# VKCOM/YouTokenToMe

Hardware: NVIDIA B200
Metric: encode throughput, 1M x 128 B synthetic sentences, vocab 32k (higher is better)
Workload: dtype u8/u32

## Files before the change

youtokentome_b200/csrc/encode.cu:

```cuda
#include <algorithm>
#include <cstdlib>
#include <cstring>

#include "common.cuh"

using namespace yt;

namespace {

constexpr int32_t EMPTY_SLOT = -1;
constexpr uint32_t NO_RANK = 0xffffffffu;

struct RuleTab {
  const uint4 *slots;
  uint32_t mask;
};

__device__ __forceinline__ uint32_t rule_rank(const RuleTab &rt, uint32_t a, uint32_t b, uint32_t *z) {
  if ((a | b) & UNK_FLAG) return NO_RANK;
  uint32_t h = rule_hash(a, b) & rt.mask;
  while (true) {
    uint4 s = __ldg(rt.slots + h);
    if (s.x == a && s.y == b) { *z = s.w; return s.z; }
    if (s.x == 0xffffffffu) return NO_RANK;
    h = (h + 1) & rt.mask;
  }
}

struct EncArgs {
  const uint8_t *bytes;
  const uint64_t *offs;
  uint64_t n_sent;
  int32_t *slots;
  uint32_t *ranks;
  uint32_t *aux;
  uint32_t *word_pos;
  uint32_t *word_sent;
// ... 134 lines not shown
  }
}

constexpr int FIND_VEC_CACHE = 8;
__device__ __forceinline__ uint32_t find_vec_word(const uint8_t *s, int64_t p, int64_t lo, int64_t hi, int64_t n_total) {
  if (p + 4 <= lo) return 0x20202020u;
  if (p >= hi) return 0u;
  uint32_t w = 0;
  if (p >= 0 && p + 4 <= n_total) w = *reinterpret_cast<const uint32_t *>(s + p);
  else
    for (int k = 0; k < 4; k++)
      if (p + k >= 0 && p + k < n_total) w |= (uint32_t)s[p + k] << (8 * k);
  if (p < lo || p + 4 > hi)
    for (int k = 0; k < 4; k++) {
      if (p + k < lo) w = (w & ~(0xffu << (8 * k))) | (0x20u << (8 * k));
      else if (p + k >= hi) w &= ~(0xffu << (8 * k));
    }
  return w;
}
__device__ __forceinline__ uint32_t swar_eq(uint32_t w, uint32_t v4) {
  const uint32_t t = w ^ v4;
  return ~(((t & 0x7f7f7f7fu) + 0x7f7f7f7fu) | t | 0x7f7f7f7fu);
}
__device__ __forceinline__ uint32_t swar_space(uint32_t w) {
  const uint32_t b7 = w & 0x7f7f7f7fu;
  const uint32_t ge9 = b7 + 0x77777777u, ge14 = b7 + 0x72727272u;
  return (swar_eq(w, 0x20202020u) | (ge9 & ~ge14 & ~w)) & 0x80808080u;
}
__device__ __forceinline__ uint32_t swar_mask4(uint32_t hi) {
  const uint32_t m = hi >> 7;
  return (m | (m >> 7) | (m >> 14) | (m >> 21)) & 15u;
}
__device__ __forceinline__ uint32_t find_vec_flags(const uint8_t *s, int64_t p, int64_t lo, int64_t hi, int64_t n_total,
                                                   unsigned lane) {
  const uint32_t c = find_vec_word(s, p, lo, hi, n_total);
  uint32_t pv = __shfl_up_sync(0xffffffffu, c, 1), nx = __shfl_down_sync(0xffffffffu, c, 1);
  if (lane == 0) pv = find_vec_word(s, p - 4, lo, hi, n_total);
  if (lane == 31) nx = find_vec_word(s, p + 4, lo, hi, n_total);
  uint32_t inside = 15u;
  if (p < lo) inside &= lo - p >= 4 ? 0u : 15u << (uint32_t)(lo - p);
  if (p + 4 > hi) inside &= hi <= p ? 0u : 15u >> (uint32_t)(p + 4 - hi);
  if (!((swar_eq(pv, 0xe2e2e2e2u) | swar_eq(c, 0xe2e2e2e2u) | swar_eq(nx, 0xe2e2e2e2u)) & 0x80808080u)) {
    const uint32_t sp = swar_mask4(swar_space(c)), sp_prev = swar_mask4(swar_space(pv)) >> 3;
    return ((sp << 1) | sp_prev) & ~sp & inside & 15u;
  }
  const uint64_t X = (uint64_t)pv | ((uint64_t)c << 32), Y = (uint64_t)c | ((uint64_t)nx << 32);
  uint32_t f = 0;
#pragma unroll
  for (int k = 0; k < 4; k++) {
    const uint32_t t = (uint32_t)(X >> (8 * (1 + k))), u = (uint32_t)(Y >> (8 * k));
    const bool before = is_space_byte((uint8_t)(t >> 16)) || (t & 0xffffffu) == 0x8196e2u;
    const bool at = is_space_byte((uint8_t)u) || (u & 0xffffffu) == 0x8196e2u;
    if (before && !at) f |= 1u << k;
  }
  return f & inside;
}
constexpr int FIND_SPW = 4;
__global__ void __launch_bounds__(256) find_words_vec_kernel(EncArgs a) {
  __shared__ unsigned long long s_cnt[8 * FIND_SPW], s_base;
  const unsigned lane = threadIdx.x & 31, wid = threadIdx.x >> 5;
  const uint64_t o0 = a.offs[0];
  const int64_t n_total = (int64_t)(a.offs[a.n_sent] - o0);
  const int64_t mis = (int64_t)(reinterpret_cast<uintptr_t>(a.bytes) & 3u);
  constexpr uint64_t PER_ROUND = 8 * FIND_SPW;
  for (uint64_t g = (uint64_t)blockIdx.x * PER_ROUND; g < a.n_sent; g += (uint64_t)gridDim.x * PER_ROUND) {
    int64_t lo[FIND_SPW], hi[FIND_SPW], start[FIND_SPW];
    uint32_t cnt[FIND_SPW];
    uint32_t cache = 0;
    constexpr int CPS = FIND_VEC_CACHE / FIND_SPW;
#pragma unroll
    for (int q = 0; q < FIND_SPW; q++) {
      const uint64_t s = g + (uint64_t)wid * FIND_SPW + q;
      lo[q] = hi[q] = start[q] = 0;
      cnt[q] = 0;
      if (s < a.n_sent) {
        lo[q] = (int64_t)(a.offs[s] - o0);
        hi[q] = (int64_t)(a.offs[s + 1] - o0);
        start[q] = lo[q] - ((lo[q] + mis) & 3);
        uint32_t mine = 0;
        int j = 0;
        for (int64_t pw = start[q]; pw < hi[q]; pw += 128, j++) {
          const uint32_t f = find_vec_flags(a.bytes, pw + 4 * lane, lo[q], hi[q], n_total, lane);
          if (j < CPS) cache |= f << (4 * (q * CPS + j));
          mine += __popc(f);
        }
        for (int o = 16; o > 0; o >>= 1) mine += __shfl_xor_sync(0xffffffffu, mine, o);
        cnt[q] = mine;
        if (lane == 0 && !a.direct) {
          const uint64_t base = sent_base((uint64_t)lo[q], s), len = (uint64_t)(hi[q] - lo[q]);
          a.n_ids[s] = (a.bos ? 1 : 0) + (a.eos ? 1 : 0);
          if (a.bos) a.slots[base] = a.bos_id;
          if (a.eos) a.slots[base + len + 2] = a.eos_id;
        }
      }
      if (lane == 0) s_cnt[wid * FIND_SPW + q] = cnt[q];
    }
    __syncthreads();
    if (wid == 0) {
      const unsigned long long c = s_cnt[lane];
      unsigned long long x = c;
      for (int o = 1; o < 32; o <<= 1) {
        const unsigned long long y = __shfl_up_sync(0xffffffffu, x, o);
        if ((int)lane >= o) x += y;
      }
      s_cnt[lane] = x - c;
      if (lane == 31) s_base = x ? atomicAdd(a.n_words, x) : 0ull;
    }
    __syncthreads();
#pragma unroll
    for (int q = 0; q < FIND_SPW; q++) {
      const uint64_t s = g + (uint64_t)wid * FIND_SPW + q;
      if (s >= a.n_sent) continue;
      unsigned long long idx = s_base + s_cnt[wid * FIND_SPW + q];
      if (lane == 0 && a.direct) { a.sent_wbase[s] = (uint32_t)idx; a.sent_wcnt[s] = cnt[q]; }
      if (!cnt[q]) continue;
      const unsigned below = (1u << lane) - 1u;
      int j = 0;
      for (int64_t pw = start[q]; pw < hi[q]; pw += 128, j++) {
        const int64_t p = pw + 4 * lane;
        const uint32_t f = j < CPS ? (cache >> (4 * (q * CPS + j))) & 15u : find_vec_flags(a.bytes, p, lo[q], hi[q], n_total, lane);
        const unsigned b0 = __ballot_sync(0xffffffffu, f & 1u), b1 = __ballot_sync(0xffffffffu, f & 2u),
                       b2 = __ballot_sync(0xffffffffu, f & 4u), b3 = __ballot_sync(0xffffffffu, f & 8u);
        const unsigned all_below = __popc(b0 & below) + __popc(b1 & below) + __popc(b2 & below) + __popc(b3 & below);
        unsigned long long i = idx + all_below;
#pragma unroll
        for (int k = 0; k < 4; k++)
          if ((f >> k) & 1u) {
            a.word_pos[i] = (uint32_t)(p + k);
            a.word_sent[i] = (uint32_t)s;
            i++;
          }
        idx += __popc(b0) + __popc(b1) + __popc(b2) + __popc(b3);
      }
    }
    __syncthreads();
  }
}

template <bool DROPOUT>
__global__ void __launch_bounds__(128) encode_words_kernel(EncArgs a, uint64_t n_words) {
  constexpr uint32_t LOCAL_W = 40;
  const uint64_t stride = (uint64_t)gridDim.x * blockDim.x;
  const uint64_t o0 = a.offs[0];
  const RuleTab rt = a.rt;
  auto rank = [&](uint32_t x, uint32_t y, uint32_t *z) { return rule_rank(rt, x, y, z); };
  for (uint64_t w = (uint64_t)blockIdx.x * blockDim.x + threadIdx.x; w < n_words; w += stride) {
    const uint64_t p0 = a.word_pos[w], s = a.word_sent[w];
    const uint64_t lo = a.offs[s] - o0, hi = a.offs[s + 1] - o0;
    const uint64_t slot0 = sent_base(lo, s) + 1 + (p0 - lo);
    int32_t *t = a.slots + slot0;
    uint64_t q = p0;
    uint32_t l;
    while (q < hi && !space_at(a.bytes, q, hi, &l)) q++;
// ... 249 lines not shown
      }
    }
    if (!no_unit && a.space_id == 0) {
      const bool drop = t[0] == 0;
      __syncthreads();
      if (drop) {
        for (uint32_t b0 = 0; b0 + 1 < n; b0 += LONG_T) {
          const uint32_t i = b0 + threadIdx.x;
          const uint32_t v = i + 1 < n ? t[i + 1] : 0u;
          __syncthreads();
          if (i + 1 < n) t[i] = v;
          __syncthreads();
        }
        n -= 1;
      }
    }
    const uint32_t n_out = no_unit ? 0 : n;
    for (uint32_t i = threadIdx.x; i < (a.direct ? n_out : owned); i += LONG_T) {
      const uint32_t v = t[i];
      t[i] = i < n_out ? ((v & UNK_FLAG) ? (uint32_t)a.unk_id : v) : (uint32_t)EMPTY_SLOT;
    }
    if (threadIdx.x == 0) {
      if (n_out && !a.direct) atomicAdd(a.n_ids + s, (unsigned long long)n_out);
      if (ll.n_tok) ll.n_tok[ll.item[w]] = n_out;
    }
    __syncthreads();
  }
}

constexpr unsigned long long DEDUP_EMPTY = ~0ull;
constexpr uint32_t DEDUP_PROBES = 8;
struct DedupArgs {
  unsigned long long *tab;
  uint32_t mask;
  uint32_t *rep;
  uint32_t *n_tok;
  uint32_t *list;
  unsigned long long *n_list;
  uint32_t weak_tag;
};

__global__ void __launch_bounds__(128) dedup_words_kernel(EncArgs a, uint64_t n_words, DedupArgs d) {
  const unsigned lane = threadIdx.x & 31;
  const uint64_t stride = (uint64_t)gridDim.x * blockDim.x;
  const uint64_t o0 = a.offs[0];
  for (uint64_t w0 = (uint64_t)blockIdx.x * blockDim.x + (threadIdx.x & ~31u); w0 < n_words; w0 += stride) {
    const uint64_t w = w0 + lane;
    bool is_rep = false;
    if (w < n_words) {
      const uint64_t p0 = a.word_pos[w], hi = a.offs[(uint64_t)a.word_sent[w] + 1] - o0;
      uint64_t q = p0, h = 0xcbf29ce484222325ull;
      uint32_t l;
      while (q < hi && !space_at(a.bytes, q, hi, &l)) { h = (h ^ a.bytes[q]) * 0x100000001b3ull; q++; }
      const uint64_t len = q - p0;
      h = mix64(h);
      const uint32_t tag = d.weak_tag ? 7u : (uint32_t)(h >> 32);
      const unsigned long long mine = ((unsigned long long)tag << 32) | (uint32_t)w;
      uint32_t idx = (uint32_t)h & d.mask, r = (uint32_t)w;
      is_rep = true;
      for (uint32_t k = 0; k < DEDUP_PROBES; k++, idx = (idx + 1) & d.mask) {
        unsigned long long cur = *(volatile unsigned long long *)(d.tab + idx);
        if (cur == DEDUP_EMPTY) {
          cur = atomicCAS(d.tab + idx, DEDUP_EMPTY, mine);
          if (cur == DEDUP_EMPTY) break;
        }
        if ((uint32_t)(cur >> 32) != tag) continue;
        const uint32_t w2 = (uint32_t)cur;
        const uint64_t p2 = a.word_pos[w2], hi2 = a.offs[(uint64_t)a.word_sent[w2] + 1] - o0;
        bool same = true;
        for (uint64_t i = 0; i < len; i++)
          if (p2 + i >= hi2 || a.bytes[p2 + i] != a.bytes[p0 + i]) { same = false; break; }
        if (same && p2 + len < hi2 && !space_at(a.bytes, p2 + len, hi2, &l)) same = false;
        if (same) { r = w2; is_rep = false; break; }
      }
      d.rep[w] = r;
    }
    const unsigned m = __ballot_sync(0xffffffffu, is_rep);
    if (m) {
      unsigned long long base = 0;
      if (lane == 0) base = atomicAdd(d.n_list, (unsigned long long)__popc(m));
      base = __shfl_sync(0xffffffffu, base, 0);
      if (is_rep) d.list[base + __popc(m & ((1u << lane) - 1))] = (uint32_t)w;
    }
  }
}

__global__ void __launch_bounds__(128) encode_rep_words_kernel(EncArgs a, DedupArgs d, LongList ll) {
  constexpr uint32_t LOCAL_W = 40;
  const uint64_t stride = (uint64_t)gridDim.x * blockDim.x;
  const uint64_t o0 = a.offs[0];
  const RuleTab rt = a.rt;
  auto rank = [&](uint32_t x, uint32_t y, uint32_t *z) { return rule_rank(rt, x, y, z); };
  const unsigned long long n_list = *d.n_list;
  for (uint64_t i = (uint64_t)blockIdx.x * blockDim.x + threadIdx.x; i < n_list; i += stride) {
    const uint32_t w = d.list[i];
    const uint64_t p0 = a.word_pos[w], s = a.word_sent[w];
    const uint64_t lo = a.offs[s] - o0, hi = a.offs[s + 1] - o0;
    const uint64_t slot0 = p0 + 3 * s + 1;
    int32_t *t = a.slots + slot0;
    uint64_t q = p0;
    uint32_t l;
    while (q < hi && !space_at(a.bytes, q, hi, &l)) q++;
    uint32_t owned = (uint32_t)(q - p0) + 1, n;
    if (ll.cap && owned > LONG_W) {
      const unsigned long long k = atomicAdd(ll.n, 1ull);
      if (k < ll.cap) { ll.pos[k] = (uint32_t)p0; ll.sent[k] = (uint32_t)s; ll.end[k] = (uint32_t)q; ll.item[k] = w; continue; }
    }
    if (owned <= LOCAL_W) {
      int32_t lt[LOCAL_W];
      uint32_t lr[LOCAL_W];
      n = encode_word(a.bytes, p0, lo, hi, a.cp2id, a.space_id, rank, nullptr, 0, a.seed, a.first_sentence + s, lt, lr,
                      nullptr, &owned);
      for (uint32_t k = 0; k < n; k++) t[k] = ((uint32_t)lt[k] & UNK_FLAG) ? a.unk_id : lt[k];
    } else {
      n = encode_word(a.bytes, p0, lo, hi, a.cp2id, a.space_id, rank, nullptr, 0, a.seed, a.first_sentence + s, t,
                      a.ranks + slot0, nullptr, &owned);
      for (uint32_t k = 0; k < n; k++)
        if ((uint32_t)t[k] & UNK_FLAG) t[k] = a.unk_id;
      if (!a.direct)
        for (uint32_t k = n; k < owned; k++) t[k] = EMPTY_SLOT;
    }
    d.n_tok[w] = n;
    if (n && !a.direct) atomicAdd(a.n_ids + s, (unsigned long long)n);
  }
}

__global__ void __launch_bounds__(256) copy_word_ids_kernel(EncArgs a, uint64_t n_words, DedupArgs d) {
  const uint64_t stride = (uint64_t)gridDim.x * blockDim.x;
  for (uint64_t w = (uint64_t)blockIdx.x * blockDim.x + threadIdx.x; w < n_words; w += stride) {
    const uint32_t r = d.rep[w];
    if (r == (uint32_t)w) continue;
    const uint32_t n = d.n_tok[r];
    if (!n) continue;
    const uint64_t s = a.word_sent[w];
    const int32_t *src = a.slots + ((uint64_t)a.word_pos[r] + 3ull * a.word_sent[r] + 1);
    int32_t *dst = a.slots + ((uint64_t)a.word_pos[w] + 3ull * s + 1);
    for (uint32_t k = 0; k < n; k++) dst[k] = src[k];
    atomicAdd(a.n_ids + s, (unsigned long long)n);
  }
}

__global__ void __launch_bounds__(256) sentence_ids_kernel(EncArgs a, const uint32_t *__restrict__ rep) {
  const unsigned lane = threadIdx.x & 31;
  const uint64_t warp = ((uint64_t)blockIdx.x * blockDim.x + threadIdx.x) >> 5;
  const uint64_t nwarps = ((uint64_t)gridDim.x * blockDim.x) >> 5;
  for (uint64_t s = warp; s < a.n_sent; s += nwarps) {
    const uint32_t w0 = a.sent_wbase[s], nw = a.sent_wcnt[s];
    uint32_t sum = 0;
    for (uint32_t i = lane; i < nw; i += 32) {
      const uint32_t w = w0 + i;
      sum += a.n_tok[rep ? rep[w] : w];
    }
    for (int o = 16; o > 0; o >>= 1) sum += __shfl_xor_sync(0xffffffffu, sum, o);
    if (lane == 0) a.n_ids[s] = (unsigned long long)sum + (a.bos ? 1 : 0) + (a.eos ? 1 : 0);
  }
}

__global__ void __launch_bounds__(256) emit_ids_kernel(EncArgs a, const uint32_t *__restrict__ rep,
                                                       const unsigned long long *__restrict__ out_off, int32_t *__restrict__ out) {
  const unsigned lane = threadIdx.x & 31;
  const uint64_t warp = ((uint64_t)blockIdx.x * blockDim.x + threadIdx.x) >> 5;
  const uint64_t nwarps = ((uint64_t)gridDim.x * blockDim.x) >> 5;
  for (uint64_t s = warp; s < a.n_sent; s += nwarps) {
    const uint32_t w0 = a.sent_wbase[s], nw = a.sent_wcnt[s];
    const unsigned long long ob = out_off[s], total = a.n_ids[s];
    auto at = [&](unsigned long long j) { return ob + (a.reverse ? total - 1 - j : j); };
    if (lane == 0) {
      if (a.bos) out[at(0)] = a.bos_id;
      if (a.eos) out[at(total - 1)] = a.eos_id;
    }
    unsigned long long pos = a.bos ? 1 : 0;
    for (uint32_t i0 = 0; i0 < nw; i0 += 32) {
      const uint32_t i = i0 + lane;
      uint32_t r = 0, n = 0;
      if (i < nw) {
        r = rep ? rep[w0 + i] : w0 + i;
        n = a.n_tok[r];
      }
      uint32_t x = n;
      for (int o = 1; o < 32; o <<= 1) {
        const uint32_t y = __shfl_up_sync(0xffffffffu, x, o);
        if ((int)lane >= o) x += y;
      }
      const uint32_t all = __shfl_sync(0xffffffffu, x, 31);
      if (n) {
        const int32_t *src = a.slots + ((uint64_t)a.word_pos[r] + 3ull * a.word_sent[r] + 1);
        const unsigned long long first = pos + (x - n);
        for (uint32_t k = 0; k < n; k++) out[at(first + k)] = src[k];
      }
      pos += all;
    }
  }
}

__global__ void __launch_bounds__(256) gather_ids_kernel(EncArgs a, const unsigned long long *__restrict__ out_off,
                                                         int32_t *__restrict__ out) {
  const unsigned lane = threadIdx.x & 31;
  const uint64_t warp = ((uint64_t)blockIdx.x * blockDim.x + threadIdx.x) >> 5;
  const uint64_t nwarps = ((uint64_t)gridDim.x * blockDim.x) >> 5;
  const uint64_t o0 = a.offs[0];
  for (uint64_t s = warp; s < a.n_sent; s += nwarps) {
    const uint64_t lo = a.offs[s] - o0, len = a.offs[s + 1] - o0 - lo;
    const uint64_t base = sent_base(lo, s);
    const unsigned long long ob = out_off[s], cnt = a.n_ids[s];
    unsigned long long done = 0;
    for (uint64_t i0 = 0; i0 < len + 3; i0 += 32) {
      uint64_t i = i0 + lane;
      int32_t v = i < len + 3 ? a.slots[base + i] : EMPTY_SLOT;
      unsigned m = __ballot_sync(0xffffffffu, v != EMPTY_SLOT);
      if (v != EMPTY_SLOT) {
        unsigned long long k = done + __popc(m & ((1u << lane) - 1));
        out[ob + (a.reverse ? cnt - 1 - k : k)] = v;
      }
      done += __popc(m);
    }
  }
}

__global__ void __launch_bounds__(256) add_base_kernel(unsigned long long *__restrict__ off, uint64_t n, unsigned long long base) {
// ... 39 lines not shown
  const uint64_t max_words = n_bytes / 2 + n_sent + 8;
  YT_CUDA(c, e->wpos.reserve(max_words * 4));
  YT_CUDA(c, e->wsent.reserve(max_words * 4));
  YT_CUDA(c, e->nids.reserve((n_sent + 1) * 8));
  YT_CUDA(c, e->out_off.reserve((n_sent + 2) * 8));
  YT_CUDA(c, e->counter.reserve(64));
  YT_CUDA(c, cudaMemsetAsync(e->counter.p, 0, 64, c->stream));
  EncArgs a;
  a.bytes = d_bytes; a.offs = d_offs; a.n_sent = n_sent;
  a.slots = e->slots.as<int32_t>(); a.ranks = e->ranks.as<uint32_t>();
  a.aux = dropout > 0 ? e->aux.as<uint32_t>() : nullptr;
  a.word_pos = e->wpos.as<uint32_t>(); a.word_sent = e->wsent.as<uint32_t>();
  a.n_words = e->counter.as<unsigned long long>();
  a.n_ids = e->nids.as<unsigned long long>();
  a.cp2id = enc->cp2id.as<uint32_t>();
  a.rt.slots = enc->rules.as<uint4>(); a.rt.mask = enc->rule_mask;
  a.space_id = enc->space_id;
  a.unk_id = enc->unk; a.bos_id = enc->bos; a.eos_id = enc->eos;
  a.bos = bos; a.eos = eos; a.reverse = reverse;
  a.drop_thresh = dropout <= 0 ? 0 : (uint64_t)(dropout * 4294967296.0);
  a.seed = seed; a.first_sentence = first_sentence;
  *out_n = 0;
  auto *d_total = e->counter.as<unsigned long long>() + 1;
  if (n_sent == 0) return 0;
  ytc::timer_begin(c, "encode");
  const bool plain = std::getenv("YTTM_ENC_PLAIN") != nullptr;
  const bool zlin = enc->zlin_ok && std::getenv("YTTM_ENC_ZLIN") != nullptr;
  const bool want_bucketed = std::getenv("YTTM_ENC_BUCKETED") != nullptr;
  const bool dedup = a.drop_thresh == 0 && (std::getenv("YTTM_ENC_DEDUP") != nullptr || (!plain && !zlin && !want_bucketed));
  const bool longw = a.drop_thresh == 0 && (std::getenv("YTTM_ENC_LONG") != nullptr || !plain);
  const bool bucketed = !dedup && (zlin || want_bucketed || (longw && std::getenv("YTTM_ENC_LONG") != nullptr));
  const bool find_vec = std::getenv("YTTM_ENC_FIND_VEC") || !(plain || std::getenv("YTTM_ENC_FIND_CACHED"));
  const bool direct = find_vec && !plain && !bucketed && !std::getenv("YTTM_ENC_SLOTS") && !std::getenv("YTTM_ENC_FIND_CACHED");
  a.direct = direct ? 1 : 0;
  a.sent_wbase = a.sent_wcnt = a.n_tok = nullptr;
  if (direct) {
    YT_CUDA(c, e->swb.reserve((n_sent + 1) * 4));
    YT_CUDA(c, e->swc.reserve((n_sent + 1) * 4));
    a.sent_wbase = e->swb.as<uint32_t>();
    a.sent_wcnt = e->swc.as<uint32_t>();
  }
  {
    ytc::timer_begin(c, "enc_find");
    if (!direct) YT_CUDA(c, cudaMemsetAsync(a.slots, 0xff, n_slots * 4, c->stream));
    if (find_vec) {
      const uint64_t blocks = std::min<uint64_t>((n_sent + 8 * FIND_SPW - 1) / (8 * FIND_SPW), (uint64_t)c->n_sm * 8);
      find_words_vec_kernel<<<(unsigned)std::max<uint64_t>(blocks, 1), 256, 0, c->stream>>>(a);
    } else {
      const uint64_t blocks = std::min<uint64_t>((n_sent + 7) / 8, (uint64_t)c->n_sm * 8);
      if (std::getenv("YTTM_ENC_FIND_CACHED")) find_words_cached_kernel<<<(unsigned)std::max<uint64_t>(blocks, 1), 256, 0, c->stream>>>(a);
      else find_words_kernel<<<(unsigned)std::max<uint64_t>(blocks, 1), 256, 0, c->stream>>>(a);
    }
    ytc::timer_end(c, "enc_find");
    c->launches++;
  }
  unsigned long long n_words = 0;
  YT_CUDA(c, cudaMemcpyAsync(&n_words, a.n_words, 8, cudaMemcpyDeviceToHost, c->stream));
  YT_CUDA(c, cudaStreamSynchronize(c->stream));
  const uint32_t *d_rep = nullptr;
  if (n_words) {
    uint64_t blocks = std::min<uint64_t>((n_words + 127) / 128, (uint64_t)c->n_sm * 16);
    ytc::timer_begin(c, "enc_words");
    LongList ll{nullptr, nullptr, nullptr, nullptr, nullptr, nullptr, 0};
    if (longw && (dedup || bucketed)) {
      const uint32_t cap = (uint32_t)(n_bytes / LONG_W + 16);
      YT_CUDA(c, e->longw.reserve((size_t)cap * 16 + 16));
      ll.n = e->longw.as<unsigned long long>();
      ll.pos = reinterpret_cast<uint32_t *>(ll.n + 2);
      ll.sent = ll.pos + cap;
      ll.end = ll.sent + cap;
      ll.item = ll.end + cap;
      ll.cap = cap;
      YT_CUDA(c, cudaMemsetAsync(ll.n, 0, 8, c->stream));
    }
    c->timers["enc_variant"].ms = (float)((dedup ? 8 : (ll.cap ? 4 : 0) + (zlin ? 2 : 0) + (bucketed ? 1 : 0)) + (direct ? 16 : 0));
    if (direct || dedup) YT_CUDA(c, e->dd_ntok.reserve(n_words * 4 + 16));
    a.n_tok = direct ? e->dd_ntok.as<uint32_t>() : nullptr;
    if (dedup) {
      uint64_t tslots = std::max<uint64_t>(ytc::pow2ceil(std::min<uint64_t>(n_words, 1ull << 20) * 2), 1024);
      if (const char *env = std::getenv("YTTM_ENC_DEDUP_SLOTS")) tslots = ytc::pow2ceil((uint64_t)std::max(1, std::atoi(env)));
      YT_CUDA(c, e->dd_tab.reserve(tslots * 8));
      YT_CUDA(c, e->dd_rep.reserve(n_words * 4 + 16));
      YT_CUDA(c, e->dd_list.reserve(n_words * 4 + 16));
      DedupArgs d;
      d.tab = e->dd_tab.as<unsigned long long>(); d.mask = (uint32_t)(tslots - 1);
      d.rep = e->dd_rep.as<uint32_t>(); d.n_tok = e->dd_ntok.as<uint32_t>(); d.list = e->dd_list.as<uint32_t>();
      d.n_list = e->counter.as<unsigned long long>() + 2;
      d.weak_tag = std::getenv("YTTM_ENC_DEDUP_WEAKTAG") != nullptr;
      d_rep = d.rep;
      YT_CUDA(c, cudaMemsetAsync(d.tab, 0xff, tslots * 8, c->stream));
      ytc::timer_begin(c, "enc_dedup");
      dedup_words_kernel<<<(unsigned)blocks, 128, 0, c->stream>>>(a, n_words, d);
      ytc::timer_end(c, "enc_dedup");
      ytc::timer_begin(c, "enc_rep");
      if (ll.cap) ll.n_tok = d.n_tok;
      encode_rep_words_kernel<<<(unsigned)blocks, 128, 0, c->stream>>>(a, d, ll);
      if (ll.cap) {
        encode_long_words_kernel<<<(unsigned)c->n_sm, LONG_T, 0, c->stream>>>(a, ll);
        c->launches++;
      }
      ytc::timer_end(c, "enc_rep");
      if (!direct) {
        ytc::timer_begin(c, "enc_copy");
        copy_word_ids_kernel<<<(unsigned)std::min<uint64_t>((n_words + 255) / 256, (uint64_t)c->n_sm * 8), 256, 0, c->stream>>>(a, n_words, d);
        ytc::timer_end(c, "enc_copy");
        c->launches++;
      }
      c->launches++;
    } else if (bucketed) {
      const unsigned wb = (unsigned)std::min<uint64_t>((n_words + BUCKET_WINDOW - 1) / BUCKET_WINDOW, (uint64_t)c->n_sm * 16);
      if (zlin) {
        if (a.drop_thresh) encode_words_bucketed_kernel<true, true><<<wb, 128, 0, c->stream>>>(a, n_words, enc->zlin, ll);
        else encode_words_bucketed_kernel<false, true><<<wb, 128, 0, c->stream>>>(a, n_words, enc->zlin, ll);
      } else if (a.drop_thresh) encode_words_bucketed_kernel<true, false><<<wb, 128, 0, c->stream>>>(a, n_words, enc->zlin, ll);
      else encode_words_bucketed_kernel<false, false><<<wb, 128, 0, c->stream>>>(a, n_words, enc->zlin, ll);
      if (ll.cap) {
        encode_long_words_kernel<<<(unsigned)c->n_sm, LONG_T, 0, c->stream>>>(a, ll);
        c->launches++;
      }
    } else if (a.drop_thresh) encode_words_kernel<true><<<(unsigned)blocks, 128, 0, c->stream>>>(a, n_words);
    else encode_words_kernel<false><<<(unsigned)blocks, 128, 0, c->stream>>>(a, n_words);
    ytc::timer_end(c, "enc_words");
    c->launches++;
  }
  const uint64_t sblocks = std::max<uint64_t>(std::min<uint64_t>((n_sent + 7) / 8, (uint64_t)c->n_sm * 8), 1);
  if (direct) {
    ytc::timer_begin(c, "enc_count");
    sentence_ids_kernel<<<(unsigned)sblocks, 256, 0, c->stream>>>(a, d_rep);
    ytc::timer_end(c, "enc_count");
    c->launches++;
  }
  ytc::timer_begin(c, "enc_scan");
  if (yttm_device_scan_u64(c, a.n_ids, n_sent, e->out_off.as<unsigned long long>(), d_total)) return 1;
  ytc::timer_end(c, "enc_scan");
  unsigned long long total = 0;
  YT_CUDA(c, cudaMemcpyAsync(&total, d_total, 8, cudaMemcpyDeviceToHost, c->stream));
  YT_CUDA(c, cudaMemcpyAsync(e->out_off.as<unsigned long long>() + n_sent, d_total, 8, cudaMemcpyDeviceToDevice,
                             c->stream));
  YT_CUDA(c, cudaStreamSynchronize(c->stream));
  YT_CUDA(c, e->out_ids.reserve((total + 8) * 4));
  {
    ytc::timer_begin(c, "enc_gather");
    if (direct) emit_ids_kernel<<<(unsigned)sblocks, 256, 0, c->stream>>>(a, d_rep, e->out_off.as<unsigned long long>(), e->out_ids.as<int32_t>());
    else gather_ids_kernel<<<(unsigned)sblocks, 256, 0, c->stream>>>(a, e->out_off.as<unsigned long long>(), e->out_ids.as<int32_t>());
    ytc::timer_end(c, "enc_gather");
    c->launches++;
  }
  ytc::timer_end(c, "encode");
  YT_CUDA(c, cudaGetLastError());
  *out_n = total;
  return 0;
}

}

extern "C" {

int yttm_enc_create(yttm_ctx *c, const uint32_t *char_cp, const uint32_t *char_id, uint64_t n_chars,
                    const uint32_t *rules_xyz, uint64_t n_rules, int unk_id, int pad_id, int bos_id, int eos_id,
                    yttm_enc **out) {
  *out = nullptr;
  YT_CUDA(c, cudaSetDevice(c->device));
  yttm_enc *e = new yttm_enc();
  e->ctx = c;
  e->unk = unk_id; e->pad = pad_id; e->bos = bos_id; e->eos = eos_id;
  std::vector<uint32_t> tab(CP_LIMIT, NO_ID);
  bool have_space = false;
  for (uint64_t i = 0; i < n_chars; i++) {
    if (char_cp[i] >= CP_LIMIT) { delete e; YT_FAIL(c, "model: code point out of range"); }
    tab[char_cp[i]] = char_id[i];
    if (char_cp[i] == SPACE_CP) { e->space_id = char_id[i]; have_space = true; }
  }
  if (!have_space) { delete e; YT_FAIL(c, "model: U+2581 missing from char2id"); }
  uint64_t per_rule = 2;
  if (const char *env = std::getenv("YTTM_ENC_RULE_SLOTS")) per_rule = (uint64_t)std::min(64, std::max(2, std::atoi(env)));
  uint64_t cap = std::max<uint64_t>(ytc::pow2ceil(n_rules * per_rule + 2), 1024);
  std::vector<uint4> slots(cap, make_uint4(0xffffffffu, 0xffffffffu, 0xffffffffu, 0));
  for (uint64_t i = 0; i < n_rules; i++) {
    uint32_t x = rules_xyz[3 * i], y = rules_xyz[3 * i + 1], z = rules_xyz[3 * i + 2];
    uint64_t h = rule_hash(x, y) & (cap - 1);
// ... 151 lines not shown
```

Baseline: 401.1.

## Fuse word finding with hash dedup and drop host syncs in encode

Adds a find_dedup_words kernel that locates word starts and ends per sentence and immediately inserts each word into a 16-byte hash table (tag, len, pos, sent) using 128-bit atomicCAS, queueing words per warp in shared memory. The point is to skip the separate dedup pass, the round trip through word_pos/word_sent arrays, and the host readback of n_words. Downstream rep/emit kernels read word position and length directly from the table entry. The output buffer is now sized from n_slots, which moves the host sync on the total id count to after the gather. Costs are higher shared memory and register pressure, 128-bit CAS contention, and a larger table.

New measurement: 380.7, median of 6. 0.949x the previous value.

```diff
diff --git a/youtokentome_b200/csrc/encode.cu b/youtokentome_b200/csrc/encode.cu
--- a/youtokentome_b200/csrc/encode.cu
+++ b/youtokentome_b200/csrc/encode.cu
@@ -3,6 +3,9 @@
 #include <cstring>
 
 #include "common.cuh"
+#ifdef YT_SIMT_EMU
+#include <atomic>
+#endif
 
 using namespace yt;
 
@@ -203,7 +206,7 @@
   return (m | (m >> 7) | (m >> 14) | (m >> 21)) & 15u;
 }
 __device__ __forceinline__ uint32_t find_vec_flags(const uint8_t *s, int64_t p, int64_t lo, int64_t hi, int64_t n_total,
-                                                   unsigned lane) {
+                                                   unsigned lane, uint32_t *sp_out) {
   const uint32_t c = find_vec_word(s, p, lo, hi, n_total);
   uint32_t pv = __shfl_up_sync(0xffffffffu, c, 1), nx = __shfl_down_sync(0xffffffffu, c, 1);
   if (lane == 0) pv = find_vec_word(s, p - 4, lo, hi, n_total);
@@ -213,17 +216,20 @@
   if (p + 4 > hi) inside &= hi <= p ? 0u : 15u >> (uint32_t)(p + 4 - hi);
   if (!((swar_eq(pv, 0xe2e2e2e2u) | swar_eq(c, 0xe2e2e2e2u) | swar_eq(nx, 0xe2e2e2e2u)) & 0x80808080u)) {
     const uint32_t sp = swar_mask4(swar_space(c)), sp_prev = swar_mask4(swar_space(pv)) >> 3;
+    *sp_out = sp & inside;
     return ((sp << 1) | sp_prev) & ~sp & inside & 15u;
   }
   const uint64_t X = (uint64_t)pv | ((uint64_t)c << 32), Y = (uint64_t)c | ((uint64_t)nx << 32);
-  uint32_t f = 0;
+  uint32_t f = 0, sp = 0;
 #pragma unroll
   for (int k = 0; k < 4; k++) {
     const uint32_t t = (uint32_t)(X >> (8 * (1 + k))), u = (uint32_t)(Y >> (8 * k));
     const bool before = is_space_byte((uint8_t)(t >> 16)) || (t & 0xffffffu) == 0x8196e2u;
     const bool at = is_space_byte((uint8_t)u) || (u & 0xffffffu) == 0x8196e2u;
     if (before && !at) f |= 1u << k;
-  }
+    if (at) sp |= 1u << k;
+  }
+  *sp_out = sp & inside;
   return f & inside;
 }
 constexpr int FIND_SPW = 4;
@@ -251,7 +257,8 @@
         uint32_t mine = 0;
         int j = 0;
         for (int64_t pw = start[q]; pw < hi[q]; pw += 128, j++) {
-          const uint32_t f = find_vec_flags(a.bytes, pw + 4 * lane, lo[q], hi[q], n_total, lane);
+          uint32_t sp;
+          const uint32_t f = find_vec_flags(a.bytes, pw + 4 * lane, lo[q], hi[q], n_total, lane, &sp);
           if (j < CPS) cache |= f << (4 * (q * CPS + j));
           mine += __popc(f);
         }
@@ -289,7 +296,8 @@
       int j = 0;
       for (int64_t pw = start[q]; pw < hi[q]; pw += 128, j++) {
         const int64_t p = pw + 4 * lane;
-        const uint32_t f = j < CPS ? (cache >> (4 * (q * CPS + j))) & 15u : find_vec_flags(a.bytes, p, lo[q], hi[q], n_total, lane);
+        uint32_t sp;
+        const uint32_t f = j < CPS ? (cache >> (4 * (q * CPS + j))) & 15u : find_vec_flags(a.bytes, p, lo[q], hi[q], n_total, lane, &sp);
         const unsigned b0 = __ballot_sync(0xffffffffu, f & 1u), b1 = __ballot_sync(0xffffffffu, f & 2u),
                        b2 = __ballot_sync(0xffffffffu, f & 4u), b3 = __ballot_sync(0xffffffffu, f & 8u);
         const unsigned all_below = __popc(b0 & below) + __popc(b1 & below) + __popc(b2 & below) + __popc(b3 & below);
@@ -605,13 +613,27 @@
 constexpr uint32_t DEDUP_PROBES = 8;
 struct DedupArgs {
   unsigned long long *tab;
+  uint4 *tab16;
   uint32_t mask;
   uint32_t *rep;
   uint32_t *n_tok;
   uint32_t *list;
   unsigned long long *n_list;
   uint32_t weak_tag;
+  uint32_t diag;
 };
+
+__device__ __forceinline__ void rep_word(const EncArgs &a, const DedupArgs &d, uint32_t r, uint64_t *p0, uint64_t *s) {
+  if (d.tab16 && r <= d.mask) {
+    const uint4 e = d.tab16[r];
+    *p0 = e.z;
+    *s = e.w;
+    return;
+  }
+  const uint32_t w = d.tab16 ? r - (d.mask + 1) : r;
+  *p0 = a.word_pos[w];
+  *s = a.word_sent[w];
+}
 
 __global__ void __launch_bounds__(128) dedup_words_kernel(EncArgs a, uint64_t n_words, DedupArgs d) {
   const unsigned lane = threadIdx.x & 31;
@@ -658,6 +680,216 @@
   }
 }
 
+constexpr uint32_t FD_Q = 128;
+constexpr uint32_t FD_NONE = 0xffffffffu;
+
+struct WordChunks {
+  const uint8_t *s;
+  const uint32_t *w;
+  int64_t pos, n_total;
+  uint32_t sh;
+  bool fast;
+  __device__ __forceinline__ WordChunks(const uint8_t *s_, uint32_t pos_, uint32_t len, int64_t n, int64_t mis)
+      : s(s_), pos(pos_), n_total(n) {
+    const uint32_t o = (uint32_t)((pos + mis) & 3);
+    const int64_t pa = pos - o;
+    sh = 8 * o;
+    w = reinterpret_cast<const uint32_t *>(s + pa);
+    fast = pa >= 0 && pa + 4 * (int64_t)((len + 3) / 4 + 1) <= n_total;
+  }
+  __device__ __forceinline__ uint32_t chunk(uint32_t i) const {
+    if (fast) return (uint32_t)((((uint64_t)w[i + 1] << 32) | w[i]) >> sh);
+    uint32_t c = 0;
+#pragma unroll 1
+    for (int k = 0; k < 4; k++) {
+      const int64_t q = pos + 4 * (int64_t)i + k;
+      if (q < n_total) c |= (uint32_t)s[q] << (8 * k);
+    }
+    return c;
+  }
+};
+__device__ __forceinline__ uint32_t tail_mask(uint32_t left) { return left >= 4 ? 0xffffffffu : 0xffffffffu >> (8 * (4 - left)); }
+
+__device__ __forceinline__ uint4 cas128(uint4 *p, uint4 cmp, uint4 val) {
+#ifdef YT_SIMT_EMU
+  static std::atomic_flag lock = ATOMIC_FLAG_INIT;
+  while (lock.test_and_set(std::memory_order_acquire)) {}
+  volatile uint32_t *q = reinterpret_cast<volatile uint32_t *>(p);
+  const uint4 old = make_uint4(q[0], q[1], q[2], q[3]);
+  if (old.x == cmp.x && old.y == cmp.y && old.z == cmp.z && old.w == cmp.w) {
+    q[0] = val.x; q[1] = val.y; q[2] = val.z; q[3] = val.w;
+  }
+  lock.clear(std::memory_order_release);
+  return old;
+#else
+  return atomicCAS(p, cmp, val);
+#endif
+}
+
+__device__ __forceinline__ uint32_t fd_resolve(const EncArgs &a, const DedupArgs &d, int64_t n_total, int64_t mis,
+                                            uint32_t pos, uint32_t len, uint32_t sent, uint32_t occ, bool *is_new) {
+  if (d.diag & 1) { *is_new = true; a.word_pos[occ] = pos; a.word_sent[occ] = sent; return d.mask + 1 + occ; }
+  const uint32_t n_chunks = (len + 3) / 4;
+  const WordChunks x(a.bytes, pos, len, n_total, mis);
+  uint64_t h = 0x9e3779b97f4a7c15ull ^ len;
+#pragma unroll 4
+  for (uint32_t i = 0; i < n_chunks; i++) h = (h ^ (x.chunk(i) & tail_mask(len - 4 * i))) * 0xff51afd7ed558ccdull;
+  h = mix64(h);
+  const uint32_t tag = d.weak_tag ? 7u : (uint32_t)(h >> 33);
+  const uint4 mine = make_uint4(tag, len, pos, sent), empty = make_uint4(FD_NONE, FD_NONE, FD_NONE, FD_NONE);
+  uint32_t idx = (uint32_t)h & d.mask;
+  *is_new = true;
+  for (uint32_t k = 0; k < DEDUP_PROBES; k++, idx = (idx + 1) & d.mask) {
+    uint4 e = __ldcg(d.tab16 + idx);
+    if (e.x == FD_NONE || e.y == FD_NONE || e.z == FD_NONE || e.w == FD_NONE) {
+      e = cas128(d.tab16 + idx, empty, mine);
+      if (e.x == FD_NONE && e.y == FD_NONE && e.z == FD_NONE && e.w == FD_NONE) return idx;
+    }
+    if (e.x != tag || e.y != len) continue;
+    if (d.diag & 2) { *is_new = false; return idx; }
+    const WordChunks y(a.bytes, e.z, len, n_total, mis);
+    uint32_t diff = 0;
+#pragma unroll 4
+    for (uint32_t i = 0; i < n_chunks; i++) diff |= (x.chunk(i) ^ y.chunk(i)) & tail_mask(len - 4 * i);
+    if (!diff) { *is_new = false; return idx; }
+  }
+  a.word_pos[occ] = pos;
+  a.word_sent[occ] = sent;
+  return d.mask + 1 + occ;
+}
+
+__global__ void __launch_bounds__(256, 3) find_dedup_words_kernel(EncArgs a, DedupArgs d) {
+  __shared__ unsigned long long s_cnt[8 * FIND_SPW], s_base;
+  __shared__ uint32_t s_n[8 * FIND_SPW];
+  __shared__ uint32_t q_pos[8][FD_Q], q_len[8][FD_Q], q_occ[8][FD_Q], q_sent[8][FD_Q];
+  const unsigned lane = threadIdx.x & 31, wid = threadIdx.x >> 5;
+  const unsigned below = (1u << lane) - 1u;
+  const uint64_t o0 = a.offs[0];
+  const int64_t n_total = (int64_t)(a.offs[a.n_sent] - o0);
+  const int64_t mis = (int64_t)(reinterpret_cast<uintptr_t>(a.bytes) & 3u);
+  uint32_t qh = 0, qn = 0;
+  auto drain = [&](bool all) {
+    while (qn >= 32 || (all && qn)) {
+      const uint32_t take = min(qn, 32u);
+      bool is_new = false;
+      uint32_t r = 0;
+      if (lane < take) {
+        const uint32_t k = (qh + lane) & (FD_Q - 1);
+        const uint32_t occ = q_occ[wid][k];
+        r = fd_resolve(a, d, n_total, mis, q_pos[wid][k], q_len[wid][k], q_sent[wid][k], occ, &is_new);
+        d.rep[occ] = r;
+      }
+      const unsigned m = __ballot_sync(0xffffffffu, is_new);
+      if (m) {
+        unsigned long long base = 0;
+        if (lane == 0) base = atomicAdd(d.n_list, (unsigned long long)__popc(m));
+        base = __shfl_sync(0xffffffffu, base, 0);
+        if (is_new) d.list[base + __popc(m & below)] = r;
+      }
+      qh = (qh + take) & (FD_Q - 1);
+      qn -= take;
+      __syncwarp();
+    }
+  };
+  constexpr uint64_t PER_ROUND = 8 * FIND_SPW;
+  constexpr int CPS = FIND_VEC_CACHE / FIND_SPW;
+  for (uint64_t g = (uint64_t)blockIdx.x * PER_ROUND; g < a.n_sent; g += (uint64_t)gridDim.x * PER_ROUND) {
+    uint32_t cnt[FIND_SPW];
+    uint32_t cache = 0, cache_sp = 0;
+#pragma unroll
+    for (int q = 0; q < FIND_SPW; q++) {
+      const uint64_t s = g + (uint64_t)wid * FIND_SPW + q;
+      cnt[q] = 0;
+      if (s < a.n_sent) {
+        const int64_t lo = (int64_t)(a.offs[s] - o0), hi = (int64_t)(a.offs[s + 1] - o0);
+        const int64_t start = lo - ((lo + mis) & 3);
+        uint32_t mine = 0;
+        int j = 0;
+        for (int64_t pw = start; pw < hi; pw += 128, j++) {
+          uint32_t sp;
+          const uint32_t f = find_vec_flags(a.bytes, pw + 4 * lane, lo, hi, n_total, lane, &sp);
+          if (j < CPS) {
+            cache |= f << (4 * (q * CPS + j));
+            cache_sp |= sp << (4 * (q * CPS + j));
+          }
+          mine += __popc(f);
+        }
+        for (int o = 16; o > 0; o >>= 1) mine += __shfl_xor_sync(0xffffffffu, mine, o);
+        cnt[q] = mine;
+      }
+      if (lane == 0) s_cnt[wid * FIND_SPW + q] = s_n[wid * FIND_SPW + q] = cnt[q];
+    }
+    __syncthreads();
+    if (wid == 0) {
+      const unsigned long long c = s_cnt[lane];
+      unsigned long long x = c;
+      for (int o = 1; o < 32; o <<= 1) {
+        const unsigned long long y = __shfl_up_sync(0xffffffffu, x, o);
+        if ((int)lane >= o) x += y;
+      }
+      s_cnt[lane] = x - c;
+      if (lane == 31) s_base = x ? atomicAdd(a.n_words, x) : 0ull;
+    }
+    __syncthreads();
+#pragma unroll 1
+    for (int q = 0; q < FIND_SPW; q++) {
+      const uint64_t s = g + (uint64_t)wid * FIND_SPW + q;
+      if (s >= a.n_sent) continue;
+      const unsigned long long idx0 = s_base + s_cnt[wid * FIND_SPW + q];
+      const uint32_t n_s = s_n[wid * FIND_SPW + q];
+      if (lane == 0) { a.sent_wbase[s] = (uint32_t)idx0; a.sent_wcnt[s] = n_s; }
+      if (!n_s) continue;
+      const int64_t lo = (int64_t)(a.offs[s] - o0), hi = (int64_t)(a.offs[s + 1] - o0);
+      const int64_t start = lo - ((lo + mis) & 3);
+      uint32_t after = (uint32_t)hi;
+      unsigned long long idx = idx0 + n_s;
+      const int nch = (int)((hi - start + 127) / 128);
+      for (int j = nch - 1; j >= 0; j--) {
+        const int64_t p = start + 128ll * j + 4 * lane;
+        uint32_t f, sp;
+        if (j < CPS) {
+          f = (cache >> (4 * (q * CPS + j))) & 15u;
+          sp = (cache_sp >> (4 * (q * CPS + j))) & 15u;
+        } else {
+          f = find_vec_flags(a.bytes, p, lo, hi, n_total, lane, &sp);
+        }
+        uint32_t sfx = sp ? (uint32_t)p + (uint32_t)(__ffs(sp) - 1) : FD_NONE;
+        for (int o = 1; o < 32; o <<= 1) {
+          const uint32_t y = __shfl_down_sync(0xffffffffu, sfx, o);
+          if (lane + o < 32) sfx = min(sfx, y);
+        }
+        uint32_t above = __shfl_down_sync(0xffffffffu, sfx, 1);
+        if (lane == 31) above = FD_NONE;
+        above = min(above, after);
+        after = min(after, __shfl_sync(0xffffffffu, sfx, 0));
+        const unsigned b0 = __ballot_sync(0xffffffffu, f & 1u), b1 = __ballot_sync(0xffffffffu, f & 2u),
+                       b2 = __ballot_sync(0xffffffffu, f & 4u), b3 = __ballot_sync(0xffffffffu, f & 8u);
+        const uint32_t n_chunk = __popc(b0) + __popc(b1) + __popc(b2) + __popc(b3);
+        idx -= n_chunk;
+        uint32_t rank = __popc(b0 & below) + __popc(b1 & below) + __popc(b2 & below) + __popc(b3 & below);
+#pragma unroll
+        for (int k = 0; k < 4; k++)
+          if ((f >> k) & 1u) {
+            const uint32_t later = sp & (15u << (k + 1)) & 15u;
+            const uint32_t wpos = (uint32_t)(p + k);
+            const uint32_t end = later ? (uint32_t)p + (uint32_t)(__ffs(later) - 1) : above;
+            const uint32_t slot = (qh + qn + rank) & (FD_Q - 1);
+            q_pos[wid][slot] = wpos;
+            q_len[wid][slot] = end - wpos;
+            q_occ[wid][slot] = (uint32_t)(idx + rank);
+            q_sent[wid][slot] = (uint32_t)s;
+            rank++;
+          }
+        qn += n_chunk;
+        __syncwarp();
+        drain(false);
+      }
+    }
+    __syncthreads();
+  }
+  drain(true);
+}
+
 __global__ void __launch_bounds__(128) encode_rep_words_kernel(EncArgs a, DedupArgs d, LongList ll) {
   constexpr uint32_t LOCAL_W = 40;
   const uint64_t stride = (uint64_t)gridDim.x * blockDim.x;
@@ -667,13 +899,16 @@
   const unsigned long long n_list = *d.n_list;
   for (uint64_t i = (uint64_t)blockIdx.x * blockDim.x + threadIdx.x; i < n_list; i += stride) {
     const uint32_t w = d.list[i];
-    const uint64_t p0 = a.word_pos[w], s = a.word_sent[w];
+    uint64_t p0, s;
+    rep_word(a, d, w, &p0, &s);
     const uint64_t lo = a.offs[s] - o0, hi = a.offs[s + 1] - o0;
     const uint64_t slot0 = p0 + 3 * s + 1;
     int32_t *t = a.slots + slot0;
     uint64_t q = p0;
     uint32_t l;
-    while (q < hi && !space_at(a.bytes, q, hi, &l)) q++;
+    if (d.tab16 && w <= d.mask) q += d.tab16[w].y;
+    else
+      while (q < hi && !space_at(a.bytes, q, hi, &l)) q++;
     uint32_t owned = (uint32_t)(q - p0) + 1, n;
     if (ll.cap && owned > LONG_W) {
       const unsigned long long k = atomicAdd(ll.n, 1ull);
@@ -729,7 +964,7 @@
   }
 }
 
-__global__ void __launch_bounds__(256) emit_ids_kernel(EncArgs a, const uint32_t *__restrict__ rep,
+__global__ void __launch_bounds__(256) emit_ids_kernel(EncArgs a, DedupArgs d, const uint32_t *__restrict__ rep,
                                                        const unsigned long long *__restrict__ out_off, int32_t *__restrict__ out) {
   const unsigned lane = threadIdx.x & 31;
   const uint64_t warp = ((uint64_t)blockIdx.x * blockDim.x + threadIdx.x) >> 5;
@@ -757,7 +992,9 @@
       }
       const uint32_t all = __shfl_sync(0xffffffffu, x, 31);
       if (n) {
-        const int32_t *src = a.slots + ((uint64_t)a.word_pos[r] + 3ull * a.word_sent[r] + 1);
+        uint64_t p0, s_r;
+        rep_word(a, d, r, &p0, &s_r);
+        const int32_t *src = a.slots + (p0 + 3ull * s_r + 1);
         const unsigned long long first = pos + (x - n);
         for (uint32_t k = 0; k < n; k++) out[at(first + k)] = src[k];
       }
@@ -863,6 +1100,7 @@
   const bool bucketed = !dedup && (zlin || want_bucketed || (longw && std::getenv("YTTM_ENC_LONG") != nullptr));
   const bool find_vec = std::getenv("YTTM_ENC_FIND_VEC") || !(plain || std::getenv("YTTM_ENC_FIND_CACHED"));
   const bool direct = find_vec && !plain && !bucketed && !std::getenv("YTTM_ENC_SLOTS") && !std::getenv("YTTM_ENC_FIND_CACHED");
+  const bool fused = direct && dedup;
   a.direct = direct ? 1 : 0;
   a.sent_wbase = a.sent_wcnt = a.n_tok = nullptr;
   if (direct) {
@@ -871,7 +1109,52 @@
     a.sent_wbase = e->swb.as<uint32_t>();
     a.sent_wcnt = e->swc.as<uint32_t>();
   }
-  {
+  c->timers["enc_variant"].ms = (float)((dedup ? 8 : (longw && bucketed ? 4 : 0) + (zlin ? 2 : 0) + (bucketed ? 1 : 0)) + (direct ? 16 : 0));
+  LongList ll{nullptr, nullptr, nullptr, nullptr, nullptr, nullptr, 0};
+  if (longw && (dedup || bucketed)) {
+    const uint32_t cap = (uint32_t)(n_bytes / LONG_W + 16);
+    YT_CUDA(c, e->longw.reserve((size_t)cap * 16 + 16));
+    ll.n = e->longw.as<unsigned long long>();
+    ll.pos = reinterpret_cast<uint32_t *>(ll.n + 2);
+    ll.sent = ll.pos + cap;
+    ll.end = ll.sent + cap;
+    ll.item = ll.end + cap;
+    ll.cap = cap;
+    YT_CUDA(c, cudaMemsetAsync(ll.n, 0, 8, c->stream));
+  }
+  DedupArgs d;
+  d.tab = nullptr; d.tab16 = nullptr; d.mask = 0; d.rep = d.n_tok = d.list = nullptr;
+  d.n_list = e->counter.as<unsigned long long>() + 2;
+  d.weak_tag = std::getenv("YTTM_ENC_DEDUP_WEAKTAG") != nullptr;
+  d.diag = std::getenv("YTTM_FD_DIAG") ? (uint32_t)std::atoi(std::getenv("YTTM_FD_DIAG")) : 0u;
+  const uint32_t *d_rep = nullptr;
+  if (fused) {
+    uint64_t tslots = std::max<uint64_t>(ytc::pow2ceil(std::min<uint64_t>(max_words, 1ull << 20) * 2), 1024);
+    if (const char *env = std::getenv("YTTM_ENC_DEDUP_SLOTS")) tslots = ytc::pow2ceil((uint64_t)std::max(1, std::atoi(env)));
+    YT_CUDA(c, e->dd_tab.reserve(tslots * 16));
+    YT_CUDA(c, e->dd_rep.reserve(max_words * 4));
+    YT_CUDA(c, e->dd_ntok.reserve((tslots + max_words) * 4));
+    YT_CUDA(c, e->dd_list.reserve(max_words * 4));
+    d.tab16 = e->dd_tab.as<uint4>(); d.mask = (uint32_t)(tslots - 1);
+    d.rep = e->dd_rep.as<uint32_t>(); d.n_tok = e->dd_ntok.as<uint32_t>(); d.list = e->dd_list.as<uint32_t>();
+    a.n_tok = d.n_tok;
+    d_rep = d.rep;
+    YT_CUDA(c, cudaMemsetAsync(d.tab16, 0xff, tslots * 16, c->stream));
+    ytc::timer_begin(c, "enc_find");
+    const uint64_t fblocks = std::min<uint64_t>((n_sent + 8 * FIND_SPW - 1) / (8 * FIND_SPW), (uint64_t)c->n_sm * 8);
+    find_dedup_words_kernel<<<(unsigned)std::max<uint64_t>(fblocks, 1), 256, 0, c->stream>>>(a, d);
+    ytc::timer_end(c, "enc_find");
+    ytc::timer_begin(c, "enc_rep");
+    if (ll.cap) ll.n_tok = d.n_tok;
+    const uint64_t rblocks = std::min<uint64_t>((max_words + 127) / 128, (uint64_t)c->n_sm * 16);
+    encode_rep_words_kernel<<<(unsigned)rblocks, 128, 0, c->stream>>>(a, d, ll);
+    if (ll.cap) {
+      encode_long_words_kernel<<<(unsigned)c->n_sm, LONG_T, 0, c->stream>>>(a, ll);
+      c->launches++;
+    }
+    ytc::timer_end(c, "enc_rep");
+    c->launches += 2;
+  } else {
     ytc::timer_begin(c, "enc_find");
     if (!direct) YT_CUDA(c, cudaMemsetAsync(a.slots, 0xff, n_slots * 4, c->stream));
     if (find_vec) {
@@ -884,75 +1167,58 @@
     }
     ytc::timer_end(c, "enc_find");
     c->launches++;
-  }
-  unsigned long long n_words = 0;
-  YT_CUDA(c, cudaMemcpyAsync(&n_words, a.n_words, 8, cudaMemcpyDeviceToHost, c->stream));
-  YT_CUDA(c, cudaStreamSynchronize(c->stream));
-  const uint32_t *d_rep = nullptr;
-  if (n_words) {
-    uint64_t blocks = std::min<uint64_t>((n_words + 127) / 128, (uint64_t)c->n_sm * 16);
-    ytc::timer_begin(c, "enc_words");
-    LongList ll{nullptr, nullptr, nullptr, nullptr, nullptr, nullptr, 0};
-    if (longw && (dedup || bucketed)) {
-      const uint32_t cap = (uint32_t)(n_bytes / LONG_W + 16);
-      YT_CUDA(c, e->longw.reserve((size_t)cap * 16 + 16));
-      ll.n = e->longw.as<unsigned long long>();
-      ll.pos = reinterpret_cast<uint32_t *>(ll.n + 2);
-      ll.sent = ll.pos + cap;
-      ll.end = ll.sent + cap;
-      ll.item = ll.end + cap;
-      ll.cap = cap;
-      YT_CUDA(c, cudaMemsetAsync(ll.n, 0, 8, c->stream));
-    }
-    c->timers["enc_variant"].ms = (float)((dedup ? 8 : (ll.cap ? 4 : 0) + (zlin ? 2 : 0) + (bucketed ? 1 : 0)) + (direct ? 16 : 0));
-    if (direct || dedup) YT_CUDA(c, e->dd_ntok.reserve(n_words * 4 + 16));
-    a.n_tok = direct ? e->dd_ntok.as<uint32_t>() : nullptr;
-    if (dedup) {
-      uint64_t tslots = std::max<uint64_t>(ytc::pow2ceil(std::min<uint64_t>(n_words, 1ull << 20) * 2), 1024);
-      if (const char *env = std::getenv("YTTM_ENC_DEDUP_SLOTS")) tslots = ytc::pow2ceil((uint64_t)std::max(1, std::atoi(env)));
-      YT_CUDA(c, e->dd_tab.reserve(tslots * 8));
-      YT_CUDA(c, e->dd_rep.reserve(n_words * 4 + 16));
-      YT_CUDA(c, e->dd_list.reserve(n_words * 4 + 16));
-      DedupArgs d;
-      d.tab = e->dd_tab.as<unsigned long long>(); d.mask = (uint32_t)(tslots - 1);
-      d.rep = e->dd_rep.as<uint32_t>(); d.n_tok = e->dd_ntok.as<uint32_t>(); d.list = e->dd_list.as<uint32_t>();
-      d.n_list = e->counter.as<unsigned long long>() + 2;
-      d.weak_tag = std::getenv("YTTM_ENC_DEDUP_WEAKTAG") != nullptr;
-      d_rep = d.rep;
-      YT_CUDA(c, cudaMemsetAsync(d.tab, 0xff, tslots * 8, c->stream));
-      ytc::timer_begin(c, "enc_dedup");
-      dedup_words_kernel<<<(unsigned)blocks, 128, 0, c->stream>>>(a, n_words, d);
-      ytc::timer_end(c, "enc_dedup");
-      ytc::timer_begin(c, "enc_rep");
-      if (ll.cap) ll.n_tok = d.n_tok;
-      encode_rep_words_kernel<<<(unsigned)blocks, 128, 0, c->stream>>>(a, d, ll);
-      if (ll.cap) {
-        encode_long_words_kernel<<<(unsigned)c->n_sm, LONG_T, 0, c->stream>>>(a, ll);
+    unsigned long long n_words = 0;
+    YT_CUDA(c, cudaMemcpyAsync(&n_words, a.n_words, 8, cudaMemcpyDeviceToHost, c->stream));
+    YT_CUDA(c, cudaStreamSynchronize(c->stream));
+    if (n_words) {
+      uint64_t blocks = std::min<uint64_t>((n_words + 127) / 128, (uint64_t)c->n_sm * 16);
+      ytc::timer_begin(c, "enc_words");
+      if (direct || dedup) YT_CUDA(c, e->dd_ntok.reserve(n_words * 4 + 16));
+      a.n_tok = direct ? e->dd_ntok.as<uint32_t>() : nullptr;
+      if (dedup) {
+        uint64_t tslots = std::max<uint64_t>(ytc::pow2ceil(std::min<uint64_t>(n_words, 1ull << 20) * 2), 1024);
+        if (const char *env = std::getenv("YTTM_ENC_DEDUP_SLOTS")) tslots = ytc::pow2ceil((uint64_t)std::max(1, std::atoi(env)));
+        YT_CUDA(c, e->dd_tab.reserve(tslots * 8));
+        YT_CUDA(c, e->dd_rep.reserve(n_words * 4 + 16));
+        YT_CUDA(c, e->dd_list.reserve(n_words * 4 + 16));
+        d.tab = e->dd_tab.as<unsigned long long>(); d.mask = (uint32_t)(tslots - 1);
+        d.rep = e->dd_rep.as<uint32_t>(); d.n_tok = e->dd_ntok.as<uint32_t>(); d.list = e->dd_list.as<uint32_t>();
+        d_rep = d.rep;
+        YT_CUDA(c, cudaMemsetAsync(d.tab, 0xff, tslots * 8, c->stream));
+        ytc::timer_begin(c, "enc_dedup");
+        dedup_words_kernel<<<(unsigned)blocks, 128, 0, c->stream>>>(a, n_words, d);
+        ytc::timer_end(c, "enc_dedup");
+        ytc::timer_begin(c, "enc_rep");
+        if (ll.cap) ll.n_tok = d.n_tok;
+        encode_rep_words_kernel<<<(unsigned)blocks, 128, 0, c->stream>>>(a, d, ll);
+        if (ll.cap) {
+          encode_long_words_kernel<<<(unsigned)c->n_sm, LONG_T, 0, c->stream>>>(a, ll);
+          c->launches++;
+        }
+        ytc::timer_end(c, "enc_rep");
+        if (!direct) {
+          ytc::timer_begin(c, "enc_copy");
+          copy_word_ids_kernel<<<(unsigned)std::min<uint64_t>((n_words + 255) / 256, (uint64_t)c->n_sm * 8), 256, 0, c->stream>>>(a, n_words, d);
+          ytc::timer_end(c, "enc_copy");
+          c->launches++;
+        }
         c->launches++;
-      }
-      ytc::timer_end(c, "enc_rep");
-      if (!direct) {
-        ytc::timer_begin(c, "enc_copy");
-        copy_word_ids_kernel<<<(unsigned)std::min<uint64_t>((n_words + 255) / 256, (uint64_t)c->n_sm * 8), 256, 0, c->stream>>>(a, n_words, d);
-        ytc::timer_end(c, "enc_copy");
-        c->launches++;
-      }
+      } else if (bucketed) {
+        const unsigned wb = (unsigned)std::min<uint64_t>((n_words + BUCKET_WINDOW - 1) / BUCKET_WINDOW, (uint64_t)c->n_sm * 16);
+        if (zlin) {
+          if (a.drop_thresh) encode_words_bucketed_kernel<true, true><<<wb, 128, 0, c->stream>>>(a, n_words, enc->zlin, ll);
+          else encode_words_bucketed_kernel<false, true><<<wb, 128, 0, c->stream>>>(a, n_words, enc->zlin, ll);
+        } else if (a.drop_thresh) encode_words_bucketed_kernel<true, false><<<wb, 128, 0, c->stream>>>(a, n_words, enc->zlin, ll);
+        else encode_words_bucketed_kernel<false, false><<<wb, 128, 0, c->stream>>>(a, n_words, enc->zlin, ll);
+        if (ll.cap) {
+          encode_long_words_kernel<<<(unsigned)c->n_sm, LONG_T, 0, c->stream>>>(a, ll);
+          c->launches++;
+        }
+      } else if (a.drop_thresh) encode_words_kernel<true><<<(unsigned)blocks, 128, 0, c->stream>>>(a, n_words);
+      else encode_words_kernel<false><<<(unsigned)blocks, 128, 0, c->stream>>>(a, n_words);
+      ytc::timer_end(c, "enc_words");
       c->launches++;
-    } else if (bucketed) {
-      const unsigned wb = (unsigned)std::min<uint64_t>((n_words + BUCKET_WINDOW - 1) / BUCKET_WINDOW, (uint64_t)c->n_sm * 16);
-      if (zlin) {
-        if (a.drop_thresh) encode_words_bucketed_kernel<true, true><<<wb, 128, 0, c->stream>>>(a, n_words, enc->zlin, ll);
-        else encode_words_bucketed_kernel<false, true><<<wb, 128, 0, c->stream>>>(a, n_words, enc->zlin, ll);
-      } else if (a.drop_thresh) encode_words_bucketed_kernel<true, false><<<wb, 128, 0, c->stream>>>(a, n_words, enc->zlin, ll);
-      else encode_words_bucketed_kernel<false, false><<<wb, 128, 0, c->stream>>>(a, n_words, enc->zlin, ll);
-      if (ll.cap) {
-        encode_long_words_kernel<<<(unsigned)c->n_sm, LONG_T, 0, c->stream>>>(a, ll);
-        c->launches++;
-      }
-    } else if (a.drop_thresh) encode_words_kernel<true><<<(unsigned)blocks, 128, 0, c->stream>>>(a, n_words);
-    else encode_words_kernel<false><<<(unsigned)blocks, 128, 0, c->stream>>>(a, n_words);
-    ytc::timer_end(c, "enc_words");
-    c->launches++;
+    }
   }
   const uint64_t sblocks = std::max<uint64_t>(std::min<uint64_t>((n_sent + 7) / 8, (uint64_t)c->n_sm * 8), 1);
   if (direct) {
@@ -964,19 +1230,19 @@
   ytc::timer_begin(c, "enc_scan");
   if (yttm_device_scan_u64(c, a.n_ids, n_sent, e->out_off.as<unsigned long long>(), d_total)) return 1;
   ytc::timer_end(c, "enc_scan");
-  unsigned long long total = 0;
-  YT_CUDA(c, cudaMemcpyAsync(&total, d_total, 8, cudaMemcpyDeviceToHost, c->stream));
   YT_CUDA(c, cudaMemcpyAsync(e->out_off.as<unsigned long long>() + n_sent, d_total, 8, cudaMemcpyDeviceToDevice,
                              c->stream));
-  YT_CUDA(c, cudaStreamSynchronize(c->stream));
-  YT_CUDA(c, e->out_ids.reserve((total + 8) * 4));
+  YT_CUDA(c, e->out_ids.reserve((n_slots + 8) * 4));
   {
     ytc::timer_begin(c, "enc_gather");
-    if (direct) emit_ids_kernel<<<(unsigned)sblocks, 256, 0, c->stream>>>(a, d_rep, e->out_off.as<unsigned long long>(), e->out_ids.as<int32_t>());
+    if (direct) emit_ids_kernel<<<(unsigned)sblocks, 256, 0, c->stream>>>(a, d, d_rep, e->out_off.as<unsigned long long>(), e->out_ids.as<int32_t>());
     else gather_ids_kernel<<<(unsigned)sblocks, 256, 0, c->stream>>>(a, e->out_off.as<unsigned long long>(), e->out_ids.as<int32_t>());
     ytc::timer_end(c, "enc_gather");
     c->launches++;
   }
+  unsigned long long total = 0;
+  YT_CUDA(c, cudaMemcpyAsync(&total, d_total, 8, cudaMemcpyDeviceToHost, c->stream));
+  YT_CUDA(c, cudaStreamSynchronize(c->stream));
   ytc::timer_end(c, "encode");
   YT_CUDA(c, cudaGetLastError());
   *out_n = total;
```
